# arkCyber/whisper-rust

Hardware: AMD Instinct MI355X
Metric: real-time factor (audio-sec/wall-sec), greedy, 30 s synthetic chunks (higher is better)
Workload: dtype f16 operands / f32 accumulate; 1 GPU; ggml-small-shaped synthetic F16 model, greedy best_of=1 temperature_inc=0, 1 x 30 s 16 kHz f32 chunk per GPU, PCM resident in HBM; flash_attn=False, parallelism=chunk-dp1

## Files before the change

### include/whisper_amd.h

```cpp
#ifndef WHISPER_AMD_H
#define WHISPER_AMD_H

#include <stdbool.h>
#include <stddef.h>
#include <stdint.h>

#if defined(__GNUC__)
#  define WHISPER_API __attribute__((visibility("default")))
#else
#  define WHISPER_API
#endif

#define WHISPER_SAMPLE_RATE 16000
#define WHISPER_N_FFT       400
#define WHISPER_HOP_LENGTH  160
#define WHISPER_CHUNK_SIZE  30

#ifdef __cplusplus
extern "C" {
#endif

enum ggml_log_level {
    GGML_LOG_LEVEL_NONE  = 0,
    GGML_LOG_LEVEL_DEBUG = 1,
// ... 351 lines not shown
                                      float * logits_out);

WHISPER_API void whisper_amd_rows_stats(struct whisper_state * state, long out[2]);
WHISPER_API int  whisper_amd_rows_enabled(struct whisper_state * state);
WHISPER_API void whisper_amd_qgemm_stats(struct whisper_state * state, long out[2]);
WHISPER_API void whisper_amd_few_rows_stats(struct whisper_state * state, long out[2]);
WHISPER_API int whisper_amd_rows_debug(struct whisper_context * ctx, struct whisper_state * state, int B, int token, int n_past,
                                       unsigned long long * granules_out, float * logits_out);
WHISPER_API int whisper_amd_rows_step_probe(struct whisper_context * ctx, struct whisper_state ** states, int B, int n_past, int n_iters, float * ms_per_step);
WHISPER_API int whisper_amd_decode_batch(struct whisper_context * ctx, struct whisper_state * state, const whisper_token * tokens, const int32_t * pos,
                                         const int32_t * seq_id, const int8_t * logits, int n_tokens);
WHISPER_API int whisper_amd_kv_op(struct whisper_state * state, int op, int a, int b, int p0, int p1);
WHISPER_API int whisper_amd_rows_fits(struct whisper_context * ctx, int B);
WHISPER_API int whisper_amd_rows_debug_rows(struct whisper_context * ctx, struct whisper_state ** states, int B, const int * tokens, const int * n_past,
                                            float * logits_out, unsigned * row_status_out);

WHISPER_API int whisper_amd_full_batch(struct whisper_context * ctx, struct whisper_state ** states, int n_chunks,
                                       struct whisper_full_params params, const float * const * samples, const int * n_samples);
WHISPER_API void whisper_amd_batch_stats(struct whisper_context * ctx, long * steps, long * rows);
WHISPER_API long whisper_amd_batch_one_launch(struct whisper_context * ctx);
WHISPER_API long whisper_amd_batch_served(struct whisper_context * ctx);

#define WHISPER_AMD_DTW_REFUSED   (-1)
#define WHISPER_AMD_DTW_NOT_TAKEN (-2)
#define WHISPER_AMD_DTW_HIP_ERROR (-3)
WHISPER_API int  whisper_amd_dtw_path(struct whisper_state * state, const float * qk, int n_heads, int n_tokens, int n_ctx, int n_audio_tokens,
                                      int sot_len, int medfilt_width, int where, int32_t * path_tok, int32_t * path_time, int cap);
WHISPER_API void whisper_amd_dtw_stats(struct whisper_state * state, long out[3]);
WHISPER_API void whisper_amd_dtw_timings(struct whisper_state * state, int64_t out[2]);

WHISPER_API int64_t whisper_amd_arena_read(struct whisper_context * ctx, int64_t offset, void * dst, int64_t cap);
WHISPER_API void    whisper_amd_load_stats(struct whisper_context * ctx, int64_t out[6]);

#ifdef __cplusplus
}
#endif
#endif
```

### whisper-rust_amd/csrc/wa_api.cpp

```cpp
#include "wa_internal.h"

#include <algorithm>
#include <chrono>
#include <cmath>
#include <cstdarg>
#include <cstring>
#include <regex>
#include <thread>

static void wa_log_default(ggml_log_level, const char * text, void *) { fputs(text, stderr); fflush(stderr); }
static ggml_log_callback g_log_cb = wa_log_default;
static void * g_log_ud = nullptr;

void wa_log(ggml_log_level level, const char * fmt, ...) {
    if (!g_log_cb) return;
    char buf[1024];
    va_list ap;
    va_start(ap, fmt);
    const int n = vsnprintf(buf, sizeof(buf), fmt, ap);
    va_end(ap);
    if (n < (int) sizeof(buf)) { g_log_cb(level, buf, g_log_ud); return; }
    std::vector<char> big(n + 1);
    va_start(ap, fmt);
    vsnprintf(big.data(), big.size(), fmt, ap);
    va_end(ap);
    g_log_cb(level, big.data(), g_log_ud);
}

int64_t wa_time_us() {
    return std::chrono::duration_cast<std::chrono::microseconds>(std::chrono::steady_clock::now().time_since_epoch()).count();
}

bool wa_hip_ok(hipError_t e, const char * what, const char * file, int line) {
// ... 661 lines not shown

static int64_t copy_out(whisper_state * st, const float * d_src, int64_t n, float * dst, int64_t cap) {
    if (!d_src) return -1;
    if (dst && cap > 0) {
        (void) hipSetDevice(st->ctx->device);
        (void) hipStreamSynchronize(st->stream);
        if (hipMemcpy(dst, d_src, (size_t) std::min(n, cap) * sizeof(float), hipMemcpyDeviceToHost) != hipSuccess) return -1;
    }
    return n;
}
int64_t whisper_amd_get_mel(struct whisper_state * st, float * dst, int64_t cap, int * n_len, int * n_mel) {
    if (n_len) *n_len = st->mel_n_len;
    if (n_mel) *n_mel = st->mel_n_mel;
    return copy_out(st, st->d_mel, (int64_t) st->mel_n_len * st->mel_n_mel, dst, cap);
}
int64_t whisper_amd_get_embd_enc(struct whisper_state * st, float * dst, int64_t cap) {
    if (!st->have_enc) return -1;
    return copy_out(st, st->d_embd_enc, (int64_t) st->enc_n_ctx * st->ctx->model.hp.n_audio_state, dst, cap);
}
int64_t whisper_amd_get_embd_conv(struct whisper_state * st, float * dst, int64_t cap) {
    if (!st->have_enc) return -1;
    return copy_out(st, st->d_embd_conv, (int64_t) st->enc_n_ctx * st->ctx->model.hp.n_audio_state, dst, cap);
}
void whisper_amd_gelu_table_f16(uint16_t * dst) {
    for (int i = 0; i < 65536; ++i) {
        _Float16 h; uint16_t u = (uint16_t) i; memcpy(&h, &u, 2);
        const float x = (float) h;
        const float g = 0.5f * x * (1.0f + tanhf(0.79788456080286535587989211986876f * x * (1.0f + 0.044715f * x * x)));
        _Float16 o = (_Float16) g; memcpy(&dst[i], &o, 2);
    }
}
void * whisper_amd_state_stream(struct whisper_state * st) { return (void *) st->stream; }

int whisper_amd_decoder_info(struct whisper_state * st, int j, double out[8], int32_t * ids, int max_ids) {
    if (!st || j < 0 || j >= WA_MAX_DECODERS) return -1;
    const auto & d = st->decoders[j];
    out[0] = d.failed; out[1] = d.completed; out[2] = d.has_ts; out[3] = d.seek_delta; out[4] = d.sequence.result_len;
    out[5] = d.sequence.avg_logprobs; out[6] = d.sequence.entropy; out[7] = st->no_speech_prob;
    const int n = (int) d.sequence.tokens.size();
    for (int i = 0; i < n && i < max_ids; ++i) ids[i] = d.sequence.tokens[i].id;
    return n;
}

int whisper_amd_full_batch(struct whisper_context * ctx, struct whisper_state ** states, int n_chunks, struct whisper_full_params params,
                           const float * const * samples, const int * n_samples) {
    if (!ctx || !states || n_chunks <= 0) return -1;
    std::vector<int> rc(n_chunks, 0);
    std::vector<std::thread> th;
    th.reserve(n_chunks);
    {
        wa_batch_groups groups(ctx, std::vector<whisper_state *>(states, states + n_chunks));
        for (int i = 0; i < n_chunks; ++i)
            th.emplace_back([&, i]() {
                rc[i] = whisper_full_with_state(ctx, states[i], params, samples[i], n_samples[i]);
                wa_batcher_leave(states[i]->batcher);
            });
        for (auto & t : th) t.join();
    }
    for (int r : rc) if (r != 0) return r;
    return 0;
}

}
```

### whisper-rust_amd/csrc/wa_exact.hip

```cpp
#include "wa_device.h"
#include <cstdlib>

#define EX_LD 40

template <int EPI>
__global__ __launch_bounds__(256, 2) void k_gemm_exact(const wa_f16 * __restrict__ A, int lda, const wa_f16 * __restrict__ W, int ldw,
                                                       int M, int N, int K, wa_epi e) {
    __shared__ __attribute__((aligned(16))) wa_f16 As[2][32 * EX_LD];
    __shared__ __attribute__((aligned(16))) wa_f16 Ws[2][32 * EX_LD];
    const int tid = threadIdx.x, lane = tid & 63, wave = tid >> 6;
    const int wm = wave >> 1, wn = wave & 1, li = lane >> 3, lj = lane & 7;
    const int tiles_n = (N + 31) / 32;
    const int m0 = (blockIdx.x / tiles_n) * 32, n0 = (blockIdx.x % tiles_n) * 32;

    float acc[2][2][32];
#pragma unroll
    for (int p = 0; p < 2; ++p)
#pragma unroll
        for (int q = 0; q < 2; ++q)
#pragma unroll
            for (int i = 0; i < 32; ++i) acc[p][q][i] = 0.0f;

    const int np = K & ~31, nsteps = np >> 5;
    const int lrow = (tid & 127) >> 2, lkc = tid & 3;
// ... 88 lines not shown
#pragma unroll
        for (int ks = 0; ks < 2; ++ks) {
            half8 a[2][4], w[2][4];
#pragma unroll
            for (int p = 0; p < 2; ++p)
#pragma unroll
                for (int c = 0; c < 4; ++c) a[p][c] = *(const half8 *) (&As[(wm * 16 + li * 2 + p) * 64 + (((ks * 4 + c) ^ li) * 8)]);
#pragma unroll
            for (int q = 0; q < 2; ++q)
#pragma unroll
                for (int c = 0; c < 4; ++c) w[q][c] = *(const half8 *) (&Ws[(wn * 16 + lj * 2 + q) * 64 + (((ks * 4 + c) ^ lj) * 8)]);
#pragma unroll
            for (int c = 0; c < 4; ++c)
#pragma unroll
                for (int i = 0; i < 8; ++i)
#pragma unroll
                    for (int p = 0; p < 2; ++p)
#pragma unroll
                        for (int q = 0; q < 2; ++q)
                            acc[p][q][c * 8 + i] = fmaf((float) w[q][c][i], (float) a[p][c][i], acc[p][q][c * 8 + i]);
        }
    }
    asm volatile("s_waitcnt vmcnt(0)" ::: "memory");
#undef EXD_ISSUE
#pragma unroll
    for (int p = 0; p < 2; ++p)
#pragma unroll
        for (int q = 0; q < 2; ++q) {
            const int m = m0 + wm * 16 + li * 2 + p, n = n0 + wn * 16 + lj * 2 + q;
            if (m < M && n < N) epi_store<EPI>(e, m, n, wa_tree32(acc[p][q]));
        }
}

#define MX_NST 3
#define MX_BM 32
#define MX_BN 32
#define MX_STAGE_HALFS ((MX_BM + MX_BN) * 128)
#define MX_PCS 4
__device__ __forceinline__ int mx_g(int row) { const int r = row & 15; return r ^ ((r >= 4 && r <= 11) ? 4 : 0); }

template <int EPI>
__global__ __launch_bounds__(256, 2) void k_gemm_exact_mfma(const wa_f16 * __restrict__ A, int lda, const wa_f16 * __restrict__ W, int ldw,
                                                            int M, int N, int K, wa_epi e) {
    extern __shared__ __attribute__((aligned(1024))) unsigned char mx_smem[];
    wa_f16 * S = (wa_f16 *) mx_smem;
    const int tid = threadIdx.x, lane = tid & 63, wave = __builtin_amdgcn_readfirstlane(tid >> 6);
    const int wm = wave >> 1, wn = wave & 1;
    const int tiles_m = (M + MX_BM - 1) / MX_BM, tiles_n = (N + MX_BN - 1) / MX_BN, per_xcd = (tiles_m * tiles_n + 7) >> 3;
    const int t = (blockIdx.x & 7) * per_xcd + (blockIdx.x >> 3);
    if (t >= tiles_m * tiles_n) return;
    const int bm = N > M ? t % tiles_m : t / tiles_n, bn = N > M ? t / tiles_m : t % tiles_n;
    const int m0 = bm * MX_BM, n0 = bn * MX_BN;
    A += (size_t) blockIdx.y * e.bs_a; W += (size_t) blockIdx.y * e.bs_w;

    const int prow = lane >> 4, pslot = lane & 15;
    unsigned goff[MX_PCS];
    int ldst[MX_PCS];
#pragma unroll
    for (int p = 0; p < MX_PCS; ++p) {
        const int row = 8 * wave + 4 * (p & 1) + prow;
        const int chunk = pslot ^ mx_g(row);
        goff[p] = p < 2 ? ((unsigned) min(m0 + row, M - 1) * (unsigned) lda + chunk * 8) * 2u : ((unsigned) min(n0 + row, N - 1) * (unsigned) ldw + chunk * 8) * 2u;
        ldst[p] = (p < 2 ? 0 : MX_BM * 128) + (8 * wave + 4 * (p & 1)) * 128;
    }
    const int nk = K >> 7;
    const __attribute__((address_space(1))) char * Ab = (const __attribute__((address_space(1))) char *) A, * Wb = (const __attribute__((address_space(1))) char *) W;
#define MX_ISSUE(kt_) do { const int k0_ = min((kt_), nk - 1) * 256; wa_f16 * st_ = S + ((kt_) % MX_NST) * MX_STAGE_HALFS; \
        _Pragma("unroll") for (int p = 0; p < MX_PCS; ++p) \
            __builtin_amdgcn_global_load_lds((const __attribute__((address_space(1))) void *) ((p < 2 ? Ab : Wb) + k0_ + goff[p]), (__attribute__((address_space(3))) void *) (st_ + ldst[p]), 16, 0, 0); \
        } while (0)

    f32x4 acc[32];
#pragma unroll
    for (int r = 0; r < 32; ++r) acc[r] = (f32x4){0.f, 0.f, 0.f, 0.f};
#pragma unroll
    for (int p = 0; p < MX_NST - 1; ++p) MX_ISSUE(p);

    const int fr = lane & 15, fk = lane >> 4;
    const int on = n0 + wn * 16 + fr, om = m0 + wm * 16 + 4 * fk;
    constexpr bool RES = EPI == WA_EPI_RESID || EPI == WA_EPI_CONV2;
    const wa_epi_pre pcol = epi_preload<RES ? WA_EPI_F32 : EPI>(e, 0, min(on, N - 1));
    float pres[4] = { 0.f, 0.f, 0.f, 0.f };
    if (RES) {
#pragma unroll
        for (int j = 0; j < 4; ++j) pres[j] = e.resid[(size_t) min(om + j, M - 1) * e.ldr + min(on, N - 1)];
    }
    const int ga = mx_g(fr);
    const wa_f16 * fa = S + (wm * 16 + fr) * 128, * fw = S + MX_BM * 128 + (wn * 16 + fr) * 128;

    for (int kt = 0; kt < nk; ++kt) {
        asm volatile("s_waitcnt vmcnt(%0)\n\ts_barrier" :: "n"((MX_NST - 2) * MX_PCS) : "memory");
        const int so = (kt % MX_NST) * MX_STAGE_HALFS;
#pragma unroll
        for (int hf = 0; hf < 2; ++hf) {
            half8 af[2], wf[2];
#pragma unroll
            for (int c = 0; c < 2; ++c) {
                af[c] = *(const half8 *) (fa + so + (((4 * fk + 2 * hf + c) ^ ga) * 8));
                wf[c] = *(const half8 *) (fw + so + (((4 * fk + 2 * hf + c) ^ ga) * 8));
            }
            __builtin_amdgcn_sched_barrier(0);
            if (hf == 0) {
                MX_ISSUE(kt + MX_NST - 1);
                __builtin_amdgcn_sched_barrier(0);
            }
#pragma unroll
            for (int c = 0; c < 2; ++c)
#pragma unroll
                for (int i = 0; i < 8; ++i)
                    acc[(2 * hf + c) * 8 + i] = __builtin_amdgcn_mfma_f32_16x16x4f32((float) af[c][i], (float) wf[c][i], acc[(2 * hf + c) * 8 + i], 0, 0, 0);
        }
    }
    asm volatile("s_waitcnt vmcnt(0)" ::: "memory");
#undef MX_ISSUE
    float res[4];
#pragma unroll
    for (int j = 0; j < 4; ++j) {
        float s32[32];
#pragma unroll
        for (int r = 0; r < 32; ++r) s32[r] = acc[r][j];
        res[j] = wa_tree32(s32);
    }
    if (EPI == WA_EPI_GELU_F16 || EPI == WA_EPI_CONV2) {
#pragma unroll
        for (int j = 0; j < 4; ++j) { float v = res[j]; if (e.bias) v = v + pcol.bias; res[j] = wa_gelu_nb(v, e.gelu); }
    }
    if (on >= N) return;
    if (EPI == WA_EPI_ATTN_PV) {
        const int np = e.aux0, nl = e.aux1;
        const half8 * vrow = (const half8 *) (W + (size_t) on * ldw + np);
        const wa_f16 * pl = (const wa_f16 *) e.out2 + (size_t) blockIdx.y * e.bs_o2;
        half8 vl[4];
#pragma unroll
        for (int c = 0; c < 4; ++c) vl[c] = vrow[c];
#pragma unroll
        for (int j = 0; j < 4; ++j) {
            const int m = min(om + j, M - 1);
            const half8 * prow = (const half8 *) (pl + (size_t) m * 32);
            half8 pv[4];
#pragma unroll
            for (int c = 0; c < 4; ++c) pv[c] = prow[c];
            double sumf = (double) res[j];
            float prod[32];
#pragma unroll
            for (int c = 0; c < 32; ++c) prod[c] = (float) vl[c >> 3][c & 7] * (float) pv[c >> 3][c & 7];
#pragma unroll
            for (int c = 0; c < 32; ++c) if (c < nl) sumf += (double) prod[c];
            if (om + j < M) {
                if (e.out3) ((float *) e.out3)[(size_t) (om + j) * e.ldo3 + blockIdx.y * 64 + on] = (float) sumf;
                else ((wa_f16 *) e.out)[(size_t) (om + j) * e.ldo + blockIdx.y * 64 + on] = f2h((float) sumf);
            }
        }
        return;
    }
    if (EPI == WA_EPI_ENC_QKV && on >= e.split0 && om + 3 < M) {
        unsigned short h4[4];
#pragma unroll
        for (int j = 0; j < 4; ++j) { float v = res[j]; if (e.bias) v = v + pcol.bias; h4[j] = f2h(v); }
        typedef unsigned mx_u2 __attribute__((ext_vector_type(2)));
        mx_u2 pk; pk.x = (unsigned) h4[0] | ((unsigned) h4[1] << 16); pk.y = (unsigned) h4[2] | ((unsigned) h4[3] << 16);
        *(mx_u2 *) ((wa_f16 *) e.out2 + (size_t) (on - e.split0) * e.ldo2 + om) = pk;
        return;
    }
#pragma unroll
    for (int j = 0; j < 4; ++j) {
        const int m = om + j;
        if (m >= M) continue;
        if (EPI == WA_EPI_GELU_F16) ((wa_f16 *) e.out)[(size_t) m * e.ldo + on] = f2h(res[j]);
        else if (EPI == WA_EPI_CONV2) {
            if (e.dbg) e.dbg[(size_t) m * e.ldo + on] = res[j];
            ((float *) e.out)[(size_t) m * e.ldo + on] = pres[j] + res[j];
        } else {
            wa_epi_pre pre = pcol;
            if (RES) pre.resid = pres[j];
            epi_apply<EPI>(e, m, on, res[j], pre);
        }
    }
}

template <int EPI>
static void gemm_exact_mfma_launch(hipStream_t s, const wa_f16 * A, int lda, const wa_f16 * W, int ldw, int M, int N, int K, const wa_epi & e, int batch = 1) {
    static bool attr_done = false;
    constexpr int lds = MX_NST * MX_STAGE_HALFS * 2;
    if (!attr_done) { (void) hipFuncSetAttribute((const void *) k_gemm_exact_mfma<EPI>, hipFuncAttributeMaxDynamicSharedMemorySize, lds); attr_done = true; }
    const int grid = ((((M + MX_BM - 1) / MX_BM) * ((N + MX_BN - 1) / MX_BN) + 7) / 8) * 8;
    hipLaunchKernelGGL((k_gemm_exact_mfma<EPI>), dim3(grid, batch), dim3(256), lds, s, A, lda, W, ldw, M, N, K, e);
}

void wa_launch_gemm_exact(hipStream_t s, wa_epi_mode mode, const wa_f16 * A, int lda, const wa_f16 * W, int ldw, int M, int N, int K,
                          const wa_epi & e) {
    static const bool no_mfma = getenv("WHISPER_AMD_NO_EXACT_MFMA") != nullptr;
    if (!no_mfma && K % 128 == 0 && lda % 8 == 0 && ldw % 8 == 0) {
#define WA_CASE(E) case E: gemm_exact_mfma_launch<E>(s, A, lda, W, ldw, M, N, K, e); return;
        switch (mode) {
            WA_CASE(WA_EPI_F16) WA_CASE(WA_EPI_ENC_QKV) WA_CASE(WA_EPI_GELU_F16) WA_CASE(WA_EPI_RESID)
            WA_CASE(WA_EPI_CONV2) WA_CASE(WA_EPI_F32) WA_CASE(WA_EPI_CROSS_KV) WA_CASE(WA_EPI_DEC_QKV)
            default: break;
        }
#undef WA_CASE
    }
    const int grid = ((M + 31) / 32) * ((N + 31) / 32);
    static const bool no_dma = getenv("WHISPER_AMD_NO_GEMM_DMA") != nullptr;
    const bool dma = !no_dma && K % 64 == 0 && K >= 256 && lda % 8 == 0 && ldw % 8 == 0;
#define WA_CASE(E) case E: if (dma) hipLaunchKernelGGL((k_gemm_exact_dma<E>), dim3(grid), dim3(256), 0, s, A, lda, W, ldw, M, N, K, e); \
                           else     hipLaunchKernelGGL((k_gemm_exact<E>), dim3(grid), dim3(256), 0, s, A, lda, W, ldw, M, N, K, e); break;
    switch (mode) {
        WA_CASE(WA_EPI_F16) WA_CASE(WA_EPI_ENC_QKV) WA_CASE(WA_EPI_GELU_F16) WA_CASE(WA_EPI_RESID)
        WA_CASE(WA_EPI_CONV2) WA_CASE(WA_EPI_F32) WA_CASE(WA_EPI_CROSS_KV) WA_CASE(WA_EPI_DEC_QKV)
    }
#undef WA_CASE
}

template <int LN_NPL>
__device__ __forceinline__ void wa_ln_stats(const float * __restrict__ xr, int d, float eps, int lane, float * lrow, float (&xv)[LN_NPL],
                                            float & mean, float & scale) {
    double s = 0.0, a = 0.0;
#pragma unroll
    for (int k = 0; k < LN_NPL; ++k) { const int i = lane + 64 * k; xv[k] = xr[i < d ? i : d - 1]; }
#pragma unroll
    for (int k = 0; k < LN_NPL; ++k) { const int i = lane + 64 * k; if (i < d) lrow[i] = xv[k]; else xv[k] = 0.0f; }
#pragma unroll
    for (int k = 0; k < LN_NPL; ++k) { s += (double) xv[k]; a += (double) fabsf(xv[k]); }
    s = wave_sum_d(s); a = wave_sum_d(a);
    float mean_hi;
    if (!wa_sum_bounds(s, a, d, mean, mean_hi, 1.0 / (double) d)) {
        bool same = true;
// ... 589 lines not shown
            }
            sum = __shfl(sum, lane & ~31, WAVE);
            inv = (float) (1.0 / sum);
        }
    }
    if (jq >= T) return;
    wa_f16 * prow = P + ((size_t) h * T + jq) * kvp;
    wa_f16 * plrow = p_left + ((size_t) h * T + jq) * 32;
    typedef unsigned as_u4 __attribute__((ext_vector_type(4)));
    for (int g = u; g < (kvp >> 3); g += LPR) {
        as_u4 pk = { 0u, 0u, 0u, 0u };
        const int c0 = 8 * g;
        if (c0 < np) {
            const float4 lo = *(const float4 *) (srow + c0), hi = *(const float4 *) (srow + c0 + 4);
            pk.x = (unsigned) f2h(lo.x * inv) | ((unsigned) f2h(lo.y * inv) << 16); pk.y = (unsigned) f2h(lo.z * inv) | ((unsigned) f2h(lo.w * inv) << 16);
            pk.z = (unsigned) f2h(hi.x * inv) | ((unsigned) f2h(hi.y * inv) << 16); pk.w = (unsigned) f2h(hi.z * inv) | ((unsigned) f2h(hi.w * inv) << 16);
        } else {
            for (int c = c0; c < c0 + 8 && c < T; ++c) plrow[c - np] = f2h(srow[c] * inv);
        }
        *(as_u4 *) (prow + c0) = pk;
    }
}

void wa_launch_attn_exact_mfma(hipStream_t s, const wa_f16 * qk, int ldqk, const wa_f16 * vt, int ldvt, int T, int d, int n_head, float scale,
                               wa_f16 * p, wa_f16 * p_left, int kvp, wa_f16 * out, int ldo, float * out32) {
    static bool attr_done = false;
    const int lds = AS_Q * (kvp + AS_PAD) * (int) sizeof(float);
    if (!attr_done) { (void) hipFuncSetAttribute((const void *) k_attn_scores_mfma, hipFuncAttributeMaxDynamicSharedMemorySize, 160 * 1024 - 4096); attr_done = true; }
    hipLaunchKernelGGL(k_attn_scores_mfma, dim3(n_head, (T + AS_Q - 1) / AS_Q), dim3(AS_THREADS), lds, s, qk, ldqk, d, T, scale, p, p_left, kvp);
    const int np = T & ~31;
    wa_epi e; e.out = out; e.ldo = ldo; e.out2 = p_left; e.bs_o2 = (long long) T * 32; e.aux0 = np; e.aux1 = T - np;
    e.out3 = out32; e.ldo3 = ldo;
    e.bs_a = (long long) T * kvp; e.bs_w = (long long) 64 * ldvt;
    gemm_exact_mfma_launch<WA_EPI_ATTN_PV>(s, p, kvp, vt, ldvt, T, 64, (np + 127) & ~127, e, n_head);
}

template <int NQ>
__global__ __launch_bounds__(ATT_THREADS) void k_attn_exact_mq(const wa_f16 * __restrict__ q, int ldq, const wa_f16 * __restrict__ kbase, size_t k_head_stride,
                                                               int k_row_stride, const wa_f16 * __restrict__ vbase, size_t v_head_stride, int v_row_stride,
                                                               int n_tokens, int n_kv, int kvp, const int8_t * __restrict__ mask, float scale,
                                                               wa_f16 * __restrict__ out, int ldo, float * __restrict__ qk_out,
                                                               float * __restrict__ out32, int8_t * __restrict__ q8, float * __restrict__ q8d, float * __restrict__ q8s) {
    constexpr int NW = ATT_THREADS / 64;
    extern __shared__ __attribute__((aligned(16))) unsigned char mq_smem[];
    float  * sc   = (float *) mq_smem;
    float  * gs   = sc + (size_t) NQ * kvp;
    float  * part = gs + (size_t) NQ * (kvp >> 3);
    wa_f16 * p16  = (wa_f16 *) (part + (size_t) NQ * 32 * 64);
    __shared__ float red[NQ][NW];
    __shared__ double redd[NQ][NW];
    __shared__ float s_inv[NQ];
    __shared__ __attribute__((aligned(16))) wa_f16 qs[NQ][64];

    const int tid = threadIdx.x, lane = tid & 63, wave = tid >> 6;
    const int n_head = gridDim.x;
    const int h = blockIdx.x, j0 = blockIdx.y * NQ;
    const wa_f16 * kp = kbase + (size_t) h * k_head_stride;
    const wa_f16 * vp = vbase + (size_t) h * v_head_stride;

    if (tid < 64 * NQ) { const int qi = tid >> 6, jq = min(j0 + qi, n_tokens - 1); qs[qi][tid & 63] = q[(size_t) jq * ldq + h * 64 + (tid & 63)]; }
    __syncthreads();

    float lmax[NQ];
#pragma unroll
    for (int qi = 0; qi < NQ; ++qi) lmax[qi] = -INFINITY;
    {
        const int a = tid & 3, kslot = tid >> 2;
// ... 216 lines not shown
```

### whisper-rust_amd/csrc/wa_kernels.h

```cpp
#pragma once
#include <hip/hip_runtime.h>
#include <cstdint>

typedef uint16_t wa_f16;

#define WA_ATT_MAXKV 5120

enum wa_epi_mode {
    WA_EPI_F16 = 0,
    WA_EPI_ENC_QKV,
    WA_EPI_GELU_F16,
    WA_EPI_RESID,
    WA_EPI_CONV2,
    WA_EPI_F32,
    WA_EPI_CROSS_KV,
    WA_EPI_GELU_F32,
    WA_EPI_DEC_QKV,
    WA_EPI_ATTN_PV,
};

struct wa_rowptr { wa_f16 * kv_k; wa_f16 * kv_v; const wa_f16 * cross_k; const wa_f16 * cross_v; int n_kv; int kv_head; };

struct wa_q8_rows { int8_t * qs = nullptr; float * qd = nullptr; float * qsum = nullptr; };

// ... 3 lines not shown
    void * out  = nullptr; int ldo  = 0;
    void * out2 = nullptr; int ldo2 = 0;
    void * out3 = nullptr; int ldo3 = 0;
    const float * resid = nullptr; int ldr = 0;
    float * dbg = nullptr;
    const wa_f16 * gelu = nullptr;
    int split0 = 0, split1 = 0;
    int row_off = 0;
    int aux0 = 0, aux1 = 0;
    const int * dyn = nullptr;
    long long bs_a = 0, bs_w = 0, bs_o2 = 0;
    const wa_rowptr * rowp = nullptr; long long rowp_off = 0;
};

void wa_launch_gemm(hipStream_t stream, wa_epi_mode mode, const wa_f16 * A, int lda, const wa_f16 * W, int ldw,
                    int M, int N, int K, const wa_epi & e);

void wa_launch_mel(hipStream_t stream, const float * pcm, int n_samples, const float * hann, const float * sincos,
                   const float * filters, int n_mel, int n_fft_bins, float * mel, int n_len, unsigned int * mel_max);

void wa_launch_mel_window(hipStream_t stream, const float * mel, int n_mel, int n_len, int seek, int n_frames,
                          wa_f16 * melT, int rows_total);

void wa_launch_layernorm(hipStream_t stream, const float * x, int ldx, int rows, int d, const float * w, const float * b,
                         float eps, wa_f16 * out16, int ld16, float * out32, int ld32);

void wa_launch_enc_attn(hipStream_t stream, const wa_f16 * qk, int ldqk, const wa_f16 * vt, int ldvt, int T, int d,
                        int n_head, float scale, wa_f16 * out, int ldo);

void wa_launch_dec_embed(hipStream_t stream, const int32_t * tok, const int32_t * pos, int n_tokens, int d,
                         const wa_f16 * te, const float * pe, float * x);

void wa_launch_gemm_exact(hipStream_t stream, wa_epi_mode mode, const wa_f16 * A, int lda, const wa_f16 * W, int ldw, int M, int N, int K,
                          const wa_epi & e);
void wa_launch_gemv_exact(hipStream_t stream, wa_epi_mode mode, const wa_f16 * A, int lda, const int32_t * rows, const wa_f16 * W, int ldw,
                          int M, int N, int K, const wa_epi & e);
void wa_launch_ln_gemv_exact(hipStream_t stream, wa_epi_mode mode, const float * x, int ldx, const int32_t * rows, const float * ln_w,
                             const float * ln_b, float eps, const wa_f16 * W, int ldw, int M, int N, int K, const wa_epi & e);
void wa_launch_im2col3(hipStream_t stream, const wa_f16 * src, int src_ld, int row0, int stride, int IC, int OL, wa_f16 * dst, int dst_ld);
void wa_launch_layernorm_exact(hipStream_t stream, const float * x, int ldx, int rows, int d, const float * w, const float * b, float eps,
                               wa_f16 * out16, int ld16, float * out32, int ld32, int8_t * qs = nullptr, float * qd = nullptr,
                               float * qsum = nullptr );
void wa_launch_attn_exact_mfma(hipStream_t stream, const wa_f16 * qk, int ldqk, const wa_f16 * vt, int ldvt, int T, int d, int n_head, float scale,
                               wa_f16 * p, wa_f16 * p_left, int kvp, wa_f16 * out, int ldo,
                               float * out32 = nullptr );
void wa_launch_attn_exact(hipStream_t stream, const wa_f16 * q, int ldq, const wa_f16 * kbase, size_t k_head_stride, int k_row_stride,
                          const wa_f16 * vbase, size_t v_head_stride, int v_row_stride, int n_head, int n_tokens, int n_kv, const int8_t * mask,
                          float scale, float * partial, wa_f16 * p_left, wa_f16 * out, int ldo, float * qk_out, const int * dyn_n_kv = nullptr,
                          float * out32 = nullptr ,
                          wa_q8_rows q8 = wa_q8_rows() ,
                          const wa_rowptr * rowp = nullptr, int rowp_cross = 0, long long rowp_off = 0
                          );

void wa_launch_quantize_q8_0(hipStream_t stream, const float * x, int ldx, int rows, int K, int8_t * qs, float * qd, float * qsum = nullptr);
void wa_launch_qgemm_exact(hipStream_t stream, wa_epi_mode mode, const int8_t * xq, const float * xd, int M, const int8_t * wq, const float * wd, int N, int K,
                           const wa_epi & e, const float * xs = nullptr, const float * wm = nullptr);
void wa_launch_qgemm_exact_route(hipStream_t stream, wa_epi_mode mode, const int8_t * xq, const float * xd, int M, const int8_t * wq, const float * wd, int N, int K,
                                 const wa_epi & e, const float * xs, const float * wm, int route);
int wa_qgemm_exact_kernel(wa_epi_mode mode, int M, int N, int K, const wa_epi & e, int route);
void wa_launch_ln_q8_row(hipStream_t stream, const float * x, int K, const float * w, const float * b, float eps, int8_t * qs, float * qd, float * qsum = nullptr);
void wa_launch_qgemv_gelu_q8(hipStream_t stream, const int8_t * xq, const float * xd, const int8_t * wq, const float * wd, int N, int K, const float * bias,
                             const wa_f16 * gelu, int8_t * oq, float * oqd, const float * xs = nullptr, const float * wm = nullptr, float * oqs = nullptr);
void wa_launch_dec_embed_q(hipStream_t stream, const int32_t * tok, const int32_t * pos, int n_tokens, int d, const int8_t * wq, const float * wd,
                           const float * pe, float * x, const float * wm = nullptr);

void wa_launch_quantize_q8_K(hipStream_t stream, const float * x, int ldx, int rows, int K, int8_t * qs, float * qd, int16_t * qbs);
void wa_launch_kgemm_exact(hipStream_t stream, wa_epi_mode mode, int wtype, const int8_t * xq, const float * xd, const int16_t * xbs, int M, const int8_t * wq,
// ... 14 lines not shown
```

### whisper-rust_amd/whisper_rs.py

```python
from __future__ import annotations

import ctypes as C
import os
from typing import Optional, Sequence

import numpy as np

_HERE = os.path.dirname(os.path.abspath(__file__))
PRODUCT_LIB = os.path.join(_HERE, "libwhisper.so")

WHISPER_SAMPLING_GREEDY = 0
WHISPER_SAMPLING_BEAM_SEARCH = 1

AHEADS_NONE, AHEADS_N_TOP_MOST, AHEADS_CUSTOM = 0, 1, 2


class WhisperError(RuntimeError):

    def __init__(self, msg: str, code: int = 0):
        super().__init__(msg)
        self.code = code


class whisper_ahead(C.Structure):
# ... 70 lines not shown
    _fields_ = [("beam_size", C.c_int), ("patience", C.c_float)]


class whisper_full_params(C.Structure):
    _fields_ = [
        ("strategy", C.c_int),
        ("n_threads", C.c_int), ("n_max_text_ctx", C.c_int), ("offset_ms", C.c_int), ("duration_ms", C.c_int),
        ("translate", C.c_bool), ("no_context", C.c_bool), ("no_timestamps", C.c_bool), ("single_segment", C.c_bool),
        ("print_special", C.c_bool), ("print_progress", C.c_bool), ("print_realtime", C.c_bool),
        ("print_timestamps", C.c_bool),
        ("token_timestamps", C.c_bool), ("thold_pt", C.c_float), ("thold_ptsum", C.c_float), ("max_len", C.c_int),
        ("split_on_word", C.c_bool), ("max_tokens", C.c_int),
        ("debug_mode", C.c_bool), ("audio_ctx", C.c_int),
        ("tdrz_enable", C.c_bool),
        ("suppress_regex", C.c_char_p),
        ("initial_prompt", C.c_char_p), ("prompt_tokens", C.POINTER(C.c_int32)), ("prompt_n_tokens", C.c_int),
        ("language", C.c_char_p), ("detect_language", C.c_bool),
        ("suppress_blank", C.c_bool), ("suppress_nst", C.c_bool),
        ("temperature", C.c_float), ("max_initial_ts", C.c_float), ("length_penalty", C.c_float),
        ("temperature_inc", C.c_float), ("entropy_thold", C.c_float), ("logprob_thold", C.c_float),
        ("no_speech_thold", C.c_float),
        ("greedy", _greedy),
        ("beam_search", _beam),
        ("new_segment_callback", NEW_SEGMENT_CB), ("new_segment_callback_user_data", C.c_void_p),
        ("progress_callback", PROGRESS_CB), ("progress_callback_user_data", C.c_void_p),
        ("encoder_begin_callback", ENCODER_BEGIN_CB), ("encoder_begin_callback_user_data", C.c_void_p),
        ("abort_callback", ABORT_CB), ("abort_callback_user_data", C.c_void_p),
        ("logits_filter_callback", LOGITS_FILTER_CB), ("logits_filter_callback_user_data", C.c_void_p),
        ("grammar_rules", C.c_void_p), ("n_grammar_rules", C.c_size_t), ("i_start_rule", C.c_size_t),
        ("grammar_penalty", C.c_float),
        ("vad", C.c_bool), ("vad_model_path", C.c_char_p),
        ("vad_params", whisper_vad_params),
    ]


_LIBS: dict[str, C.CDLL] = {}


def load_library(path: Optional[str] = None) -> C.CDLL:
    path = os.path.abspath(path or PRODUCT_LIB)
    if path in _LIBS:
        return _LIBS[path]
    if not os.path.exists(path):
        raise OSError(f"{path} not found - build it first (python -c 'import __graft_entry__ as g; g.build()')")
    lib = C.CDLL(path, mode=C.RTLD_LOCAL)
    P, I, F = C.c_void_p, C.c_int, C.c_float

    def proto(name, res, *args):
        fn = getattr(lib, name)
        fn.restype = res
        fn.argtypes = list(args)

    proto("whisper_context_default_params", whisper_context_params)
    proto("whisper_full_default_params", whisper_full_params, I)
    proto("whisper_init_from_file_with_params_no_state", P, C.c_char_p, whisper_context_params)
    proto("whisper_init_from_buffer_with_params_no_state", P, P, C.c_size_t, whisper_context_params)
    proto("whisper_init_state", P, P)
    proto("whisper_free", None, P)
    proto("whisper_free_state", None, P)
    proto("whisper_pcm_to_mel_with_state", I, P, P, C.POINTER(F), I, I)
    proto("whisper_set_mel_with_state", I, P, P, C.POINTER(F), I, I)
    proto("whisper_encode_with_state", I, P, P, I, I)
    proto("whisper_decode_with_state", I, P, P, C.POINTER(C.c_int32), I, I, I)
    proto("whisper_lang_auto_detect_with_state", I, P, P, I, I, C.POINTER(F))
    proto("whisper_get_logits_from_state", C.POINTER(F), P)
    proto("whisper_n_len_from_state", I, P)
# ... 51 lines not shown
    proto("whisper_vad_segments_from_samples", P, P, whisper_vad_params, C.POINTER(F), I)
    proto("whisper_vad_segments_n_segments", I, P)
    proto("whisper_vad_segments_get_segment_t0", F, P, I)
    proto("whisper_vad_segments_get_segment_t1", F, P, I)
    proto("whisper_vad_free_segments", None, P)
    proto("whisper_vad_free", None, P)
    if hasattr(lib, "whisper_amd_vad_front"):
        proto("whisper_amd_vad_front", C.c_int64, P, C.POINTER(F), I, C.POINTER(F), C.c_int64)
        proto("whisper_amd_vad_tile", I)
    if hasattr(lib, "whisper_amd_full_batch"):
        proto("whisper_amd_full_batch", I, P, C.POINTER(C.c_void_p), I, whisper_full_params, C.POINTER(C.c_void_p), C.POINTER(C.c_int))
    if hasattr(lib, "whisper_amd_rows_stats"):
        proto("whisper_amd_rows_stats", None, P, C.POINTER(C.c_long))
        proto("whisper_amd_rows_enabled", I, P)
        proto("whisper_amd_batch_one_launch", C.c_long, P)
    if hasattr(lib, "whisper_amd_decode_batch"):
        proto("whisper_amd_decode_batch", I, P, P, C.POINTER(C.c_int32), C.POINTER(C.c_int32), C.POINTER(C.c_int32), C.POINTER(C.c_int8), I)
        proto("whisper_amd_kv_op", I, P, I, I, I, I, I)
        proto("whisper_amd_rows_fits", I, P, I)
        proto("whisper_amd_rows_debug_rows", I, P, C.POINTER(C.c_void_p), I, C.POINTER(C.c_int), C.POINTER(C.c_int), C.POINTER(F), C.POINTER(C.c_uint))
    if hasattr(lib, "whisper_amd_batch_served"):
        proto("whisper_amd_batch_served", C.c_long, P)
    if hasattr(lib, "whisper_amd_dtw_path"):
        proto("whisper_amd_dtw_path", I, P, C.POINTER(F), I, I, I, I, I, I, I, C.POINTER(C.c_int32), C.POINTER(C.c_int32), I)
        proto("whisper_amd_dtw_stats", None, P, C.POINTER(C.c_long))
        proto("whisper_amd_dtw_timings", None, P, C.POINTER(C.c_int64))
    if hasattr(lib, "whisper_amd_qgemm_stats"):
        proto("whisper_amd_qgemm_stats", None, P, C.POINTER(C.c_long))
    if hasattr(lib, "whisper_amd_few_rows_stats"):
        proto("whisper_amd_few_rows_stats", None, P, C.POINTER(C.c_long))
    if hasattr(lib, "whisper_amd_arena_read"):
        proto("whisper_amd_arena_read", C.c_int64, P, C.c_int64, P, C.c_int64)
        proto("whisper_amd_load_stats", None, P, C.POINTER(C.c_int64))
    _LIBS[path] = lib
    return lib


DTW_REFUSED, DTW_NOT_TAKEN, DTW_HIP_ERROR = -1, -2, -3

_KEEP_LOG_CB = {}


def set_log_callback(lib: C.CDLL, fn=None):
    cb = LOG_CB((lambda lvl, txt, ud: None) if fn is None else (lambda lvl, txt, ud: fn(lvl, (txt or b"").decode(errors="replace"))))
    _KEEP_LOG_CB[id(lib)] = cb
    lib.whisper_log_set(cb, None)


class WhisperContextParameters:

    def __init__(self, lib: C.CDLL, use_gpu: bool = True, flash_attn: bool = False, gpu_device: int = 0,
                 dtw_preset: int = AHEADS_NONE, dtw_n_top: int = -1, dtw_heads: Sequence[tuple] = ()):
        p = lib.whisper_context_default_params()
        p.use_gpu = use_gpu
        p.flash_attn = flash_attn
        p.gpu_device = gpu_device
        if dtw_preset != AHEADS_NONE:
            p.dtw_token_timestamps = True
            p.dtw_aheads_preset = dtw_preset
            p.dtw_n_top = dtw_n_top
            if dtw_preset == AHEADS_CUSTOM:
                self._heads = (whisper_ahead * len(dtw_heads))(*[whisper_ahead(a, b) for a, b in dtw_heads])
                p.dtw_aheads.n_heads = len(dtw_heads)
                p.dtw_aheads.heads = self._heads
        self.c = p

# ... 452 lines not shown
```

Before: 366.6 x real-time.

## Make exact MFMA GEMM persistent with cross-tile prefetch and occupancy-sized grid

The exact MFMA GEMM kernel now works persistently: each workgroup walks several output tiles, including batch/head tiles, within its XCD partition. The cp.async-style LDS prefetch pipeline carries straight across tile boundaries, so the next tile's loads overlap the current tile's epilogue, and the grid is sized from occupancy times the CU count instead of one workgroup per tile. Launch bounds move from 2 to 3 workgroups per CU. It also adds a public test entry point for the kernel. The aim is to cut tail/wave-quantization and pipeline-fill costs on the encoder GEMMs, at the risk of register pressure at the higher occupancy and more complex indexing.

```diff
diff --git a/include/whisper_amd.h b/include/whisper_amd.h
--- a/include/whisper_amd.h
+++ b/include/whisper_amd.h
@@ -407,6 +407,15 @@
 WHISPER_API int64_t whisper_amd_arena_read(struct whisper_context * ctx, int64_t offset, void * dst, int64_t cap);
 WHISPER_API void    whisper_amd_load_stats(struct whisper_context * ctx, int64_t out[6]);
 
+struct whisper_amd_gemm_exact_args {
+    const void * a; const void * w;
+    const float * bias; const float * scale; const float * resid; const void * gelu;
+    void * out; void * out2;
+    int64_t bs_a, bs_w, bs_o2;
+    int32_t mode, m, n, k, lda, ldw, ldo, ldo2, ldr, split0, aux0, aux1, batch, max_wgs;
+};
+WHISPER_API int whisper_amd_gemm_exact(const struct whisper_amd_gemm_exact_args * args);
+
 #ifdef __cplusplus
 }
 #endif
diff --git a/whisper-rust_amd/csrc/wa_api.cpp b/whisper-rust_amd/csrc/wa_api.cpp
--- a/whisper-rust_amd/csrc/wa_api.cpp
+++ b/whisper-rust_amd/csrc/wa_api.cpp
@@ -1,4 +1,5 @@
 #include "wa_internal.h"
+#include "wa_kernels.h"
 
 #include <algorithm>
 #include <chrono>
@@ -726,6 +727,29 @@
 }
 void * whisper_amd_state_stream(struct whisper_state * st) { return (void *) st->stream; }
 
+int whisper_amd_gemm_exact(const struct whisper_amd_gemm_exact_args * p) {
+    if (!p || !p->a || !p->w || !p->out || p->m <= 0 || p->n <= 0 || p->k <= 0) return (int) hipErrorInvalidValue;
+    wa_epi e;
+    e.bias = p->bias; e.scale = p->scale; e.resid = p->resid; e.ldr = p->ldr; e.gelu = (const wa_f16 *) p->gelu;
+    e.out = p->out; e.ldo = p->ldo; e.out2 = p->out2; e.ldo2 = p->ldo2;
+    e.split0 = p->split0; e.aux0 = p->aux0; e.aux1 = p->aux1;
+    e.bs_a = p->bs_a; e.bs_w = p->bs_w; e.bs_o2 = p->bs_o2;
+    const wa_f16 * a = (const wa_f16 *) p->a, * w = (const wa_f16 *) p->w;
+    switch (p->mode) {
+        case WA_EPI_F16: case WA_EPI_ENC_QKV: case WA_EPI_GELU_F16: case WA_EPI_RESID: case WA_EPI_F32: case WA_EPI_CROSS_KV:
+            wa_launch_gemm_exact(nullptr, (wa_epi_mode) p->mode, a, p->lda, w, p->ldw, p->m, p->n, p->k, e, p->max_wgs);
+            break;
+        case WA_EPI_ATTN_PV:
+            if (p->n != 64 || p->k % 128 || p->lda % 8 || p->ldw % 8 || p->batch < 1 || !p->out2) return (int) hipErrorInvalidValue;
+            wa_launch_gemm_exact_pv(nullptr, a, p->lda, w, p->ldw, p->m, p->k, e, p->batch, p->max_wgs);
+            break;
+        default: return (int) hipErrorInvalidValue;
+    }
+    hipError_t err = hipGetLastError();
+    if (err == hipSuccess) err = hipStreamSynchronize(nullptr);
+    return (int) err;
+}
+
 int whisper_amd_decoder_info(struct whisper_state * st, int j, double out[8], int32_t * ids, int max_ids) {
     if (!st || j < 0 || j >= WA_MAX_DECODERS) return -1;
     const auto & d = st->decoders[j];
diff --git a/whisper-rust_amd/csrc/wa_exact.hip b/whisper-rust_amd/csrc/wa_exact.hip
--- a/whisper-rust_amd/csrc/wa_exact.hip
+++ b/whisper-rust_amd/csrc/wa_exact.hip
@@ -144,6 +144,7 @@
         }
 }
 
+#define MX_WGS 3
 #define MX_NST 3
 #define MX_BM 32
 #define MX_BN 32
@@ -151,44 +152,80 @@
 #define MX_PCS 4
 __device__ __forceinline__ int mx_g(int row) { const int r = row & 15; return r ^ ((r >= 4 && r <= 11) ? 4 : 0); }
 
+typedef const __attribute__((address_space(1))) char * mx_gptr;
+
 template <int EPI>
-__global__ __launch_bounds__(256, 2) void k_gemm_exact_mfma(const wa_f16 * __restrict__ A, int lda, const wa_f16 * __restrict__ W, int ldw,
-                                                            int M, int N, int K, wa_epi e) {
+__global__ __launch_bounds__(256, MX_WGS) void k_gemm_exact_mfma(const wa_f16 * __restrict__ A, int lda, const wa_f16 * __restrict__ W, int ldw,
+                                                                 int M, int N, int K, int batch, wa_epi e) {
     extern __shared__ __attribute__((aligned(1024))) unsigned char mx_smem[];
     wa_f16 * S = (wa_f16 *) mx_smem;
     const int tid = threadIdx.x, lane = tid & 63, wave = __builtin_amdgcn_readfirstlane(tid >> 6);
     const int wm = wave >> 1, wn = wave & 1;
-    const int tiles_m = (M + MX_BM - 1) / MX_BM, tiles_n = (N + MX_BN - 1) / MX_BN, per_xcd = (tiles_m * tiles_n + 7) >> 3;
-    const int t = (blockIdx.x & 7) * per_xcd + (blockIdx.x >> 3);
-    if (t >= tiles_m * tiles_n) return;
-    const int bm = N > M ? t % tiles_m : t / tiles_n, bn = N > M ? t / tiles_m : t % tiles_n;
-    const int m0 = bm * MX_BM, n0 = bn * MX_BN;
-    A += (size_t) blockIdx.y * e.bs_a; W += (size_t) blockIdx.y * e.bs_w;
+    const unsigned tiles_m = (M + MX_BM - 1) / MX_BM, tiles_n = (N + MX_BN - 1) / MX_BN, tiles = tiles_m * tiles_n, total = tiles * (unsigned) batch;
+    const unsigned xcd = blockIdx.x & 7, wpx = gridDim.x >> 3;
+    const unsigned first = xcd * total / 8 + (blockIdx.x >> 3), hi = (xcd + 1) * total / 8;
+    if (first >= hi) return;
+    const int mine = __builtin_amdgcn_readfirstlane((int) ((hi - first + wpx - 1) / wpx));
+    const int nk = K >> 7;
+    const bool n_longer = N > M;
+#define MX_TILE(t_, pb_, m0_, n0_) do { const unsigned pb__ = (t_) / tiles, tt_ = (t_) - pb__ * tiles; \
+        const unsigned q_ = n_longer ? tt_ / tiles_m : tt_ / tiles_n, r_ = tt_ - q_ * (n_longer ? tiles_m : tiles_n); \
+        pb_ = (int) pb__; m0_ = (int) (n_longer ? r_ : q_) * MX_BM; n0_ = (int) (n_longer ? q_ : r_) * MX_BN; } while (0)
 
     const int prow = lane >> 4, pslot = lane & 15;
-    unsigned goff[MX_PCS];
+    const unsigned pchunk16 = (unsigned) (pslot ^ mx_g(8 * wave + prow)) * 16u;
     int ldst[MX_PCS];
 #pragma unroll
-    for (int p = 0; p < MX_PCS; ++p) {
-        const int row = 8 * wave + 4 * (p & 1) + prow;
-        const int chunk = pslot ^ mx_g(row);
-        goff[p] = p < 2 ? ((unsigned) min(m0 + row, M - 1) * (unsigned) lda + chunk * 8) * 2u : ((unsigned) min(n0 + row, N - 1) * (unsigned) ldw + chunk * 8) * 2u;
-        ldst[p] = (p < 2 ? 0 : MX_BM * 128) + (8 * wave + 4 * (p & 1)) * 128;
-    }
-    const int nk = K >> 7;
-    const __attribute__((address_space(1))) char * Ab = (const __attribute__((address_space(1))) char *) A, * Wb = (const __attribute__((address_space(1))) char *) W;
-#define MX_ISSUE(kt_) do { const int k0_ = min((kt_), nk - 1) * 256; wa_f16 * st_ = S + ((kt_) % MX_NST) * MX_STAGE_HALFS; \
-        _Pragma("unroll") for (int p = 0; p < MX_PCS; ++p) \
-            __builtin_amdgcn_global_load_lds((const __attribute__((address_space(1))) void *) ((p < 2 ? Ab : Wb) + k0_ + goff[p]), (__attribute__((address_space(3))) void *) (st_ + ldst[p]), 16, 0, 0); \
+    for (int p = 0; p < MX_PCS; ++p) ldst[p] = (p < 2 ? 0 : MX_BM * 128) + (8 * wave + 4 * (p & 1)) * 128;
+    int i_t = 0, i_kt = 0, i_lm, i_ln;
+    mx_gptr i_a, i_w;
+#define MX_SEEK() do { int pb_, m0_, n0_; MX_TILE(first + (unsigned) i_t * wpx, pb_, m0_, n0_); \
+        i_a = (mx_gptr) (A + (size_t) pb_ * e.bs_a + (size_t) m0_ * lda); i_w = (mx_gptr) (W + (size_t) pb_ * e.bs_w + (size_t) n0_ * ldw); \
+        i_lm = M - 1 - m0_; i_ln = N - 1 - n0_; } while (0)
+#define MX_ISSUE(slot_) do { \
+        _Pragma("unroll") for (int p = 0; p < MX_PCS; ++p) { \
+            const int row_ = min(8 * wave + 4 * (p & 1) + prow, p < 2 ? i_lm : i_ln); \
+            const unsigned off_ = (unsigned) row_ * (unsigned) (2 * (p < 2 ? lda : ldw)) + pchunk16; \
+            __builtin_amdgcn_global_load_lds((const __attribute__((address_space(1))) void *) ((p < 2 ? i_a : i_w) + i_kt * 256 + off_), \
+                                             (__attribute__((address_space(3))) void *) (S + (slot_) + ldst[p]), 16, 0, 0); } \
+        if (++i_kt == nk) { if (i_t + 1 < mine) { ++i_t; i_kt = 0; MX_SEEK(); } else i_kt = nk - 1; } \
         } while (0)
-
+    MX_SEEK();
+#pragma unroll
+    for (int st = 0; st < MX_NST - 1; ++st) MX_ISSUE(st * MX_STAGE_HALFS);
+    int rs = 0, ws = (MX_NST - 1) * MX_STAGE_HALFS;
+
+    const int fr = lane & 15, fk = lane >> 4;
+    const unsigned fb = ((wm * 16 + fr) * 128 + ((4 * fk) ^ mx_g(fr)) * 8) * 2u;
+    const int fwd = (MX_BM * 128 + (wn - wm) * 16 * 128) * 2;
     f32x4 acc[32];
-#pragma unroll
-    for (int r = 0; r < 32; ++r) acc[r] = (f32x4){0.f, 0.f, 0.f, 0.f};
-#pragma unroll
-    for (int p = 0; p < MX_NST - 1; ++p) MX_ISSUE(p);
-
-    const int fr = lane & 15, fk = lane >> 4;
+#define MX_WAIT() asm volatile("s_waitcnt vmcnt(%0)\n\ts_barrier" :: "n"((MX_NST - 2) * MX_PCS) : "memory")
+#define MX_STAGE(FIRST_) do { \
+        _Pragma("unroll") for (int hf = 0; hf < 2; ++hf) {        \
+            half8 af[2], wf[2]; \
+            _Pragma("unroll") for (int c = 0; c < 2; ++c) { \
+                const unsigned fo_ = (fb + 2u * rs) ^ (16u * (2 * hf + c)); \
+                af[c] = *(const half8 *) (mx_smem + fo_); \
+                wf[c] = *(const half8 *) (mx_smem + fo_ + fwd); \
+            } \
+            __builtin_amdgcn_sched_barrier(0); \
+            if (hf == 0) { \
+                MX_ISSUE(ws); \
+                __builtin_amdgcn_sched_barrier(0); \
+            } \
+            _Pragma("unroll") for (int c = 0; c < 2; ++c) \
+                _Pragma("unroll") for (int i = 0; i < 8; ++i) \
+                    acc[(2 * hf + c) * 8 + i] = __builtin_amdgcn_mfma_f32_16x16x4f32((float) af[c][i], (float) wf[c][i], \
+                        (FIRST_) ? (f32x4){0.f, 0.f, 0.f, 0.f} : acc[(2 * hf + c) * 8 + i], 0, 0, 0); \
+        } \
+        ws = rs; rs = rs == (MX_NST - 1) * MX_STAGE_HALFS ? 0 : rs + MX_STAGE_HALFS; \
+        } while (0)
+
+    for (int ti = 0; ti < mine; ++ti) {
+    int pb, m0, n0;
+    MX_TILE(first + (unsigned) ti * wpx, pb, m0, n0);
+    const wa_f16 * Wp = W + (size_t) pb * e.bs_w;
+    MX_WAIT();
     const int on = n0 + wn * 16 + fr, om = m0 + wm * 16 + 4 * fk;
     constexpr bool RES = EPI == WA_EPI_RESID || EPI == WA_EPI_CONV2;
     const wa_epi_pre pcol = epi_preload<RES ? WA_EPI_F32 : EPI>(e, 0, min(on, N - 1));
@@ -197,34 +234,10 @@
 #pragma unroll
         for (int j = 0; j < 4; ++j) pres[j] = e.resid[(size_t) min(om + j, M - 1) * e.ldr + min(on, N - 1)];
     }
-    const int ga = mx_g(fr);
-    const wa_f16 * fa = S + (wm * 16 + fr) * 128, * fw = S + MX_BM * 128 + (wn * 16 + fr) * 128;
-
-    for (int kt = 0; kt < nk; ++kt) {
-        asm volatile("s_waitcnt vmcnt(%0)\n\ts_barrier" :: "n"((MX_NST - 2) * MX_PCS) : "memory");
-        const int so = (kt % MX_NST) * MX_STAGE_HALFS;
-#pragma unroll
-        for (int hf = 0; hf < 2; ++hf) {
-            half8 af[2], wf[2];
-#pragma unroll
-            for (int c = 0; c < 2; ++c) {
-                af[c] = *(const half8 *) (fa + so + (((4 * fk + 2 * hf + c) ^ ga) * 8));
-                wf[c] = *(const half8 *) (fw + so + (((4 * fk + 2 * hf + c) ^ ga) * 8));
-            }
-            __builtin_amdgcn_sched_barrier(0);
-            if (hf == 0) {
-                MX_ISSUE(kt + MX_NST - 1);
-                __builtin_amdgcn_sched_barrier(0);
-            }
-#pragma unroll
-            for (int c = 0; c < 2; ++c)
-#pragma unroll
-                for (int i = 0; i < 8; ++i)
-                    acc[(2 * hf + c) * 8 + i] = __builtin_amdgcn_mfma_f32_16x16x4f32((float) af[c][i], (float) wf[c][i], acc[(2 * hf + c) * 8 + i], 0, 0, 0);
-        }
-    }
-    asm volatile("s_waitcnt vmcnt(0)" ::: "memory");
-#undef MX_ISSUE
+    MX_STAGE(true);
+    for (int kt = 1; kt < nk; ++kt) { MX_WAIT(); MX_STAGE(false); }
+
+    do {
     float res[4];
 #pragma unroll
     for (int j = 0; j < 4; ++j) {
@@ -237,11 +250,12 @@
 #pragma unroll
         for (int j = 0; j < 4; ++j) { float v = res[j]; if (e.bias) v = v + pcol.bias; res[j] = wa_gelu_nb(v, e.gelu); }
     }
-    if (on >= N) return;
+    asm volatile("" : "+v"(res[0]), "+v"(res[1]), "+v"(res[2]), "+v"(res[3]) : "v"(pcol.bias), "v"(pcol.scale), "v"(pres[0]), "v"(pres[1]), "v"(pres[2]), "v"(pres[3]));
+    if (on >= N) break;
     if (EPI == WA_EPI_ATTN_PV) {
         const int np = e.aux0, nl = e.aux1;
-        const half8 * vrow = (const half8 *) (W + (size_t) on * ldw + np);
-        const wa_f16 * pl = (const wa_f16 *) e.out2 + (size_t) blockIdx.y * e.bs_o2;
+        const half8 * vrow = (const half8 *) (Wp + (size_t) on * ldw + np);
+        const wa_f16 * pl = (const wa_f16 *) e.out2 + (size_t) pb * e.bs_o2;
         half8 vl[4];
 #pragma unroll
         for (int c = 0; c < 4; ++c) vl[c] = vrow[c];
@@ -259,11 +273,11 @@
 #pragma unroll
             for (int c = 0; c < 32; ++c) if (c < nl) sumf += (double) prod[c];
             if (om + j < M) {
-                if (e.out3) ((float *) e.out3)[(size_t) (om + j) * e.ldo3 + blockIdx.y * 64 + on] = (float) sumf;
-                else ((wa_f16 *) e.out)[(size_t) (om + j) * e.ldo + blockIdx.y * 64 + on] = f2h((float) sumf);
-            }
-        }
-        return;
+                if (e.out3) ((float *) e.out3)[(size_t) (om + j) * e.ldo3 + pb * 64 + on] = (float) sumf;
+                else ((wa_f16 *) e.out)[(size_t) (om + j) * e.ldo + pb * 64 + on] = f2h((float) sumf);
+            }
+        }
+        break;
     }
     if (EPI == WA_EPI_ENC_QKV && on >= e.split0 && om + 3 < M) {
         unsigned short h4[4];
@@ -272,7 +286,7 @@
         typedef unsigned mx_u2 __attribute__((ext_vector_type(2)));
         mx_u2 pk; pk.x = (unsigned) h4[0] | ((unsigned) h4[1] << 16); pk.y = (unsigned) h4[2] | ((unsigned) h4[3] << 16);
         *(mx_u2 *) ((wa_f16 *) e.out2 + (size_t) (on - e.split0) * e.ldo2 + om) = pk;
-        return;
+        break;
     }
 #pragma unroll
     for (int j = 0; j < 4; ++j) {
@@ -288,22 +302,41 @@
             epi_apply<EPI>(e, m, on, res[j], pre);
         }
     }
+    } while (0);
+    }
+    asm volatile("s_waitcnt vmcnt(0)" ::: "memory");
+#undef MX_STAGE
+#undef MX_WAIT
+#undef MX_ISSUE
+#undef MX_SEEK
+#undef MX_TILE
 }
 
 template <int EPI>
-static void gemm_exact_mfma_launch(hipStream_t s, const wa_f16 * A, int lda, const wa_f16 * W, int ldw, int M, int N, int K, const wa_epi & e, int batch = 1) {
-    static bool attr_done = false;
+static void gemm_exact_mfma_launch(hipStream_t s, const wa_f16 * A, int lda, const wa_f16 * W, int ldw, int M, int N, int K, const wa_epi & e, int batch = 1,
+                                   int max_wgs = 0) {
+    static int slots = 0;
     constexpr int lds = MX_NST * MX_STAGE_HALFS * 2;
-    if (!attr_done) { (void) hipFuncSetAttribute((const void *) k_gemm_exact_mfma<EPI>, hipFuncAttributeMaxDynamicSharedMemorySize, lds); attr_done = true; }
-    const int grid = ((((M + MX_BM - 1) / MX_BM) * ((N + MX_BN - 1) / MX_BN) + 7) / 8) * 8;
-    hipLaunchKernelGGL((k_gemm_exact_mfma<EPI>), dim3(grid, batch), dim3(256), lds, s, A, lda, W, ldw, M, N, K, e);
+    if (!slots) {
+        (void) hipFuncSetAttribute((const void *) k_gemm_exact_mfma<EPI>, hipFuncAttributeMaxDynamicSharedMemorySize, lds);
+        int per_cu = 0, dev = 0, cus = 0;
+        if (hipOccupancyMaxActiveBlocksPerMultiprocessor(&per_cu, k_gemm_exact_mfma<EPI>, 256, lds) != hipSuccess || per_cu < 1) per_cu = 1;
+        if (hipGetDevice(&dev) != hipSuccess || hipDeviceGetAttribute(&cus, hipDeviceAttributeMultiprocessorCount, dev) != hipSuccess || cus < 1) cus = 256;
+        slots = per_cu * cus;
+    }
+    const long n = (long) ((M + MX_BM - 1) / MX_BM) * ((N + MX_BN - 1) / MX_BN) * batch;
+    const long rounds = (n + slots - 1) / slots;
+    const long walk = n * 20 >= rounds * slots * 19 ? rounds : (rounds > 2 ? rounds / 2 : 1);
+    long grid = (((n + walk - 1) / walk + 7) / 8) * 8;
+    if (max_wgs > 0 && grid > max_wgs) grid = max_wgs >= 8 ? (max_wgs / 8) * 8 : 8;
+    hipLaunchKernelGGL((k_gemm_exact_mfma<EPI>), dim3((unsigned) grid), dim3(256), lds, s, A, lda, W, ldw, M, N, K, batch, e);
 }
 
 void wa_launch_gemm_exact(hipStream_t s, wa_epi_mode mode, const wa_f16 * A, int lda, const wa_f16 * W, int ldw, int M, int N, int K,
-                          const wa_epi & e) {
+                          const wa_epi & e, int max_wgs) {
     static const bool no_mfma = getenv("WHISPER_AMD_NO_EXACT_MFMA") != nullptr;
     if (!no_mfma && K % 128 == 0 && lda % 8 == 0 && ldw % 8 == 0) {
-#define WA_CASE(E) case E: gemm_exact_mfma_launch<E>(s, A, lda, W, ldw, M, N, K, e); return;
+#define WA_CASE(E) case E: gemm_exact_mfma_launch<E>(s, A, lda, W, ldw, M, N, K, e, 1, max_wgs); return;
         switch (mode) {
             WA_CASE(WA_EPI_F16) WA_CASE(WA_EPI_ENC_QKV) WA_CASE(WA_EPI_GELU_F16) WA_CASE(WA_EPI_RESID)
             WA_CASE(WA_EPI_CONV2) WA_CASE(WA_EPI_F32) WA_CASE(WA_EPI_CROSS_KV) WA_CASE(WA_EPI_DEC_QKV)
@@ -959,7 +992,11 @@
     wa_epi e; e.out = out; e.ldo = ldo; e.out2 = p_left; e.bs_o2 = (long long) T * 32; e.aux0 = np; e.aux1 = T - np;
     e.out3 = out32; e.ldo3 = ldo;
     e.bs_a = (long long) T * kvp; e.bs_w = (long long) 64 * ldvt;
-    gemm_exact_mfma_launch<WA_EPI_ATTN_PV>(s, p, kvp, vt, ldvt, T, 64, (np + 127) & ~127, e, n_head);
+    wa_launch_gemm_exact_pv(s, p, kvp, vt, ldvt, T, (np + 127) & ~127, e, n_head);
+}
+
+void wa_launch_gemm_exact_pv(hipStream_t s, const wa_f16 * A, int lda, const wa_f16 * W, int ldw, int M, int K, const wa_epi & e, int batch, int max_wgs) {
+    gemm_exact_mfma_launch<WA_EPI_ATTN_PV>(s, A, lda, W, ldw, M, 64, K, e, batch, max_wgs);
 }
 
 template <int NQ>
diff --git a/whisper-rust_amd/csrc/wa_kernels.h b/whisper-rust_amd/csrc/wa_kernels.h
--- a/whisper-rust_amd/csrc/wa_kernels.h
+++ b/whisper-rust_amd/csrc/wa_kernels.h
@@ -59,7 +59,9 @@
                          const wa_f16 * te, const float * pe, float * x);
 
 void wa_launch_gemm_exact(hipStream_t stream, wa_epi_mode mode, const wa_f16 * A, int lda, const wa_f16 * W, int ldw, int M, int N, int K,
-                          const wa_epi & e);
+                          const wa_epi & e, int max_wgs = 0);
+void wa_launch_gemm_exact_pv(hipStream_t stream, const wa_f16 * A, int lda, const wa_f16 * W, int ldw, int M, int K, const wa_epi & e, int batch,
+                             int max_wgs = 0);
 void wa_launch_gemv_exact(hipStream_t stream, wa_epi_mode mode, const wa_f16 * A, int lda, const int32_t * rows, const wa_f16 * W, int ldw,
                           int M, int N, int K, const wa_epi & e);
 void wa_launch_ln_gemv_exact(hipStream_t stream, wa_epi_mode mode, const float * x, int ldx, const int32_t * rows, const float * ln_w,
diff --git a/whisper-rust_amd/whisper_rs.py b/whisper-rust_amd/whisper_rs.py
--- a/whisper-rust_amd/whisper_rs.py
+++ b/whisper-rust_amd/whisper_rs.py
@@ -126,6 +126,26 @@
         ("vad", C.c_bool), ("vad_model_path", C.c_char_p),
         ("vad_params", whisper_vad_params),
     ]
+
+
+class whisper_amd_gemm_exact_args(C.Structure):
+    _fields_ = [
+        ("a", C.c_void_p), ("w", C.c_void_p),
+        ("bias", C.c_void_p), ("scale", C.c_void_p), ("resid", C.c_void_p), ("gelu", C.c_void_p),
+        ("out", C.c_void_p), ("out2", C.c_void_p),
+        ("bs_a", C.c_int64), ("bs_w", C.c_int64), ("bs_o2", C.c_int64),
+        ("mode", C.c_int32), ("m", C.c_int32), ("n", C.c_int32), ("k", C.c_int32), ("lda", C.c_int32), ("ldw", C.c_int32),
+        ("ldo", C.c_int32), ("ldo2", C.c_int32), ("ldr", C.c_int32), ("split0", C.c_int32), ("aux0", C.c_int32), ("aux1", C.c_int32),
+        ("batch", C.c_int32), ("max_wgs", C.c_int32),
+    ]
+
+
+EPI_F16, EPI_ENC_QKV, EPI_GELU_F16, EPI_RESID, EPI_F32, EPI_CROSS_KV, EPI_ATTN_PV = 0, 1, 2, 3, 5, 6, 9
+
+
+def gemm_exact(lib: C.CDLL, **fields) -> int:
+    args = whisper_amd_gemm_exact_args(**fields)
+    return lib.whisper_amd_gemm_exact(C.byref(args))
 
 
 _LIBS: dict[str, C.CDLL] = {}
@@ -243,6 +263,8 @@
     if hasattr(lib, "whisper_amd_arena_read"):
         proto("whisper_amd_arena_read", C.c_int64, P, C.c_int64, P, C.c_int64)
         proto("whisper_amd_load_stats", None, P, C.POINTER(C.c_int64))
+    if hasattr(lib, "whisper_amd_gemm_exact"):
+        proto("whisper_amd_gemm_exact", I, C.POINTER(whisper_amd_gemm_exact_args))
     _LIBS[path] = lib
     return lib
 
```

After: 368.6 x real-time, median of 6. About the same (+0.5%).
